# Chairy-neko/TinyRayTracing

Hardware: AMD Instinct MI355X
Metric: Mrays/s (higher is better)
Workload: dtype f32; 1 GPU; example-scenes-cg22 test/back Cornell-style box (26 triangles), 1920x1080, 256 spp; scene=back, width=1920, height=1080, spp=256, triangles=26, bvh_nodes=4, bvh_builder=auto, leaf_num=8, inner_node_bytes=64, overlap_passes=False, fixed_nee=False, tiling=single GPU

## Files before the change

tinyraytracing_amd/csrc/trt_api.hip:

```cpp
#include <hip/hip_runtime.h>

#include <dlfcn.h>

#include <algorithm>
#include <cstdio>
#include <cstdlib>
#include <atomic>
#include <limits>
#include <chrono>
#include <cstring>
#include <condition_variable>
#include <memory>
#include <mutex>
#include <string>
#include <thread>
#include <vector>

#include "trt.h"
#include "trt_kernels.h"
#include "trt_wide.h"
#include "trt_oct_build.h"

using namespace trtd;

// ... 14 lines not shown
            return fail(e_ == hipErrorOutOfMemory ? TRT_ENOMEM : TRT_EHIP, std::string(#expr) + ": " + hipGetErrorString(e_)); \
    } while (0)

constexpr uint32_t MAX_TRACE_BLOCKS = 8192;
constexpr uint32_t SPILL_STRIDE = MAX_TRACE_BLOCKS * TRT_TRACE_BLOCK;
constexpr uint32_t MAX_BOUNCES = TRT_MAX_PATH_DEPTH + 2;
constexpr uint32_t COUNT_STRIDE = (MAX_BOUNCES + 2 + 1023u) & ~1023u;
constexpr uint32_t COUNT_ROW_MIN = 16;
inline uint32_t countRows(uint32_t nl) { return std::max(COUNT_ROW_MIN, (nl + 3u + 15u) & ~15u); }
inline unsigned long long* pairCounter(uint32_t* d_counts, uint32_t rows, uint32_t b) { return reinterpret_cast<unsigned long long*>(d_counts + (size_t)(rows - 2u) * COUNT_STRIDE) + b; }
static_assert(TRT_MAX_SCENE_LIGHTS <= 65535u, "counter area");
constexpr uint32_t MAX_BVH_DEPTH = 256;
#ifndef TRT_DEFAULT_NODE_KIND
#define TRT_DEFAULT_NODE_KIND 1
#endif

struct DevBuf {
    void* p = nullptr;
    size_t bytes = 0;
    int ensure(size_t need)
    {
        if (need <= bytes) return TRT_OK;
        if (p) { (void)hipFree(p); p = nullptr; bytes = 0; }
        HIPC(hipMalloc(&p, need));
        bytes = need;
        return TRT_OK;
    }
    void release()
    {
        if (p) (void)hipFree(p);
        p = nullptr;
        bytes = 0;
    }
};

}

struct trt_handle {
    int device = 0;
    SceneDev sc{};
    std::vector<void*> scene_allocs;
    std::vector<uint32_t> light_mats;
    std::vector<LightBox> light_boxes;
    uint32_t depth = 0;
    uint32_t bvh2_depth = 0;
    uint32_t shade_tabs = 0;
    uint32_t shade_pad_lds = 0;
    const void* lds_image = nullptr;
    uint32_t lds_image_bytes = 0;
    uint32_t lds_tab[5] = {0, 0, 0, 0, 0};
    int trace_impl = 3;
    bool slim_walk = false;
    bool hit8 = false;
    int node_kind = 0;
    uint32_t oct_levels = 0;
    bool dbg = false;
    uint32_t rays_per_wave = 256, fill_blocks = 2048, max_blocks = 8192;
    uint32_t traceGrid(uint32_t n) const
    {
        uint32_t b = (n + TRT_TRACE_BLOCK - 1) / TRT_TRACE_BLOCK;
        if (rays_per_wave > 64) {
            const uint32_t want = (uint32_t)(((uint64_t)n + 4ull * rays_per_wave - 1) / (4ull * rays_per_wave));
            b = std::min(b, std::max(fill_blocks, want));
        }
        b = std::min(std::max(b, 8u), std::min(max_blocks, 8192u));
        return (b + 7u) & ~7u;
    }
    uint32_t tail_n = 131072;
    DevBuf arena, spill, small_buf, out_buf, io_buf;
    size_t spill_words_per_slot = 0;
    hipStream_t slot_streams[2] = {nullptr, nullptr};
    int n_slots = 2;
    uint32_t* pinned_counts = nullptr;
    uint32_t count_rows = COUNT_ROW_MIN;
    uint32_t slot_seq[2] = {0, 0};
    int fail_at_bounce = -1;
    std::vector<hipEvent_t> events;
    ~trt_handle()
    {
        for (void* p : scene_allocs) (void)hipFree(p);
        arena.release();
        spill.release();
        small_buf.release();
        out_buf.release();
        io_buf.release();
        for (hipEvent_t e : events) (void)hipEventDestroy(e);
        for (hipStream_t st : slot_streams) if (st) (void)hipStreamDestroy(st);
        if (pinned_counts) (void)hipHostFree(pinned_counts);
    }
};

namespace {

template <class T>
int upload(trt_handle* h, const T* src, size_t count, const T** dst)
{
    void* p = nullptr;
    const size_t bytes = (std::max<size_t>(count, 1) * sizeof(T) + 15) & ~(size_t)15;
    HIPC(hipMalloc(&p, bytes));
    h->scene_allocs.push_back(p);
    if (count) HIPC(hipMemcpy(p, src, count * sizeof(T), hipMemcpyHostToDevice));
    *dst = (const T*)p;
    return TRT_OK;
}

int validateBvh(const trt_scene* s, uint32_t* depth_out, unsigned threads = 1)
// ... 106 lines not shown

bool rowSelected(const trt_params* p, int y) { return p->row_mod <= 1 || ((y / p->row_block) % p->row_mod) == p->row_rem; }

uint32_t tailGrid(uint32_t n)
{
    uint32_t b = (n + TRT_TRACE_BLOCK - 1) / TRT_TRACE_BLOCK;
    b = std::min(std::max(b, 8u), MAX_TRACE_BLOCKS);
    return (b + 7u) & ~7u;
}
struct Timer {
    trt_handle* h;
    bool on;
    size_t used = 0;
    struct Span { int k; size_t e0, e1; };
    std::vector<Span> spans{};
    static constexpr size_t RESERVED = 3;
    hipEvent_t get(size_t i)
    {
        while (h->events.size() <= i) {
            hipEvent_t e;
            if (hipEventCreate(&e) != hipSuccess) return nullptr;
            h->events.push_back(e);
        }
        return h->events[i];
    }
    size_t mark(hipStream_t stream)
    {
        hipEvent_t e = get(RESERVED + used);
        if (e) (void)hipEventRecord(e, stream);
        return RESERVED + used++;
    }
    void begin(int k, hipStream_t stream) { if (on) spans.push_back({k, mark(stream), 0}); }
    void end(hipStream_t stream) { if (on) spans.back().e1 = mark(stream); }
    template <class F>
    void launch(int k, hipStream_t stream, trt_stats& st, F&& f)
    {
        begin(k, stream);
        f();
        end(stream);
        st.launches[k]++;
    }
};

using ClosestKernel = void (*)(SceneDev, RaySource, f4*, uint32_t, uint32_t*, uint32_t, DeviceStats*, RedoList);
using ShadowKernel = void (*)(SceneDev, ShadowQueue, uint32_t, uint32_t, f4*, uint32_t*, uint32_t, DeviceStats*, uint32_t, RedoList, LightBox);
using FixKernel = void (*)(SceneDev, RaySource, f4*, const f4*, uint32_t, f4*, uint32_t*, uint32_t, RedoList, uint32_t, DeviceStats*);
using ShadeKernel = void (*)(SceneDev, ShadeArgs);
using TailKernel = void (*)(SceneDev, TailArgs);

constexpr uint32_t OCT_LDS_LEVELS = 10;
int traversalOf(const trt_handle* h) { return h->trace_impl == 0 ? 0 : (h->node_kind == 1 ? 1 : (h->depth <= 16 ? 2 : 3)); }
ClosestKernel closestKernel(const trt_handle* h, bool count, int primary)
{
    if (h->trace_impl == 0 && h->hit8) {
        const ClosestKernel s[2][3] = {
            {k_trace_closest<false, 1, false, 0, 0, 0, true, true>, k_trace_closest<false, 1, false, 0, 1, 0, true, true>, k_trace_closest<false, 1, false, 0, PRIMARY_LIST, 0, true, true>},
            {k_trace_closest<true, 1, false, 0, 0, 0, true, true>, k_trace_closest<true, 1, false, 0, 1, 0, true, true>, k_trace_closest<true, 1, false, 0, PRIMARY_LIST, 0, true, true>}};
        return s[count][primary];
    }
    const ClosestKernel k[4][2][3] = {
        {{k_trace_closest<false, 1, false, 0, 0, 0>, k_trace_closest<false, 1, false, 0, 1, 0>, k_trace_closest<false, 1, false, 0, PRIMARY_LIST, 0>},
         {k_trace_closest<true, 1, false, 0, 0, 0>, k_trace_closest<true, 1, false, 0, 1, 0>, k_trace_closest<true, 1, false, 0, PRIMARY_LIST, 0>}},
        {{k_trace_closest<false, OCT_LDS_LEVELS, true, 3, 0, 1>, k_trace_closest<false, OCT_LDS_LEVELS, true, 3, 1, 1>, k_trace_closest<false, OCT_LDS_LEVELS, true, 3, PRIMARY_LIST, 1>},
         {k_trace_closest<true, OCT_LDS_LEVELS, true, 3, 0, 1>, k_trace_closest<true, OCT_LDS_LEVELS, true, 3, 1, 1>, k_trace_closest<true, OCT_LDS_LEVELS, true, 3, PRIMARY_LIST, 1>}},
        {{k_trace_closest<false, 16, false, 3, 0, 0>, k_trace_closest<false, 16, false, 3, 1, 0>, k_trace_closest<false, 16, false, 3, PRIMARY_LIST, 0>},
         {k_trace_closest<true, 16, false, 3, 0, 0>, k_trace_closest<true, 16, false, 3, 1, 0>, k_trace_closest<true, 16, false, 3, PRIMARY_LIST, 0>}},
        {{k_trace_closest<false, TRT_LDS_STACK_MAX, true, 3, 0, 0>, k_trace_closest<false, TRT_LDS_STACK_MAX, true, 3, 1, 0>, k_trace_closest<false, TRT_LDS_STACK_MAX, true, 3, PRIMARY_LIST, 0>},
         {k_trace_closest<true, TRT_LDS_STACK_MAX, true, 3, 0, 0>, k_trace_closest<true, TRT_LDS_STACK_MAX, true, 3, 1, 0>, k_trace_closest<true, TRT_LDS_STACK_MAX, true, 3, PRIMARY_LIST, 0>}}};
    return k[traversalOf(h)][count][primary];
}
ShadowKernel shadowKernel(const trt_handle* h, bool count)
{
    if (h->trace_impl == 0 && h->slim_walk) return count ? k_trace_shadow<true, 1, false, 0, 0, true> : k_trace_shadow<false, 1, false, 0, 0, true>;
    const ShadowKernel k[4][2] = {{k_trace_shadow<false, 1, false, 0, 0>, k_trace_shadow<true, 1, false, 0, 0>},
                                  {k_trace_shadow<false, OCT_LDS_LEVELS, true, 3, 1>, k_trace_shadow<true, OCT_LDS_LEVELS, true, 3, 1>},
                                  {k_trace_shadow<false, 16, false, 3, 0>, k_trace_shadow<true, 16, false, 3, 0>},
                                  {k_trace_shadow<false, TRT_LDS_STACK_MAX, true, 3, 0>, k_trace_shadow<true, TRT_LDS_STACK_MAX, true, 3, 0>}};
    return k[traversalOf(h)][count];
}
FixKernel fixKernel(const trt_handle* h, bool shadow, int primary)
{
    const FixKernel k[4] = {k_trace_fix<false, 0, 0>, k_trace_fix<false, 1, 0>, k_trace_fix<false, PRIMARY_LIST, 0>, k_trace_fix<true, false, 0>};
    return h->trace_impl == 0 ? nullptr : k[shadow ? 3 : primary];
}
ClosestKernel queryKernel(const trt_handle* h, int query)
{
    const bool occ = query == QUERY_OCCLUDED;
    if (h->trace_impl == 0 && h->hit8 && !occ) return k_trace_query<QUERY_CLOSEST, true, 1, false, 0, 0, true, true>;
    if (h->trace_impl == 0 && h->slim_walk && occ) return k_trace_query<QUERY_OCCLUDED, true, 1, false, 0, 0, false, true>;
    const ClosestKernel k[4][2] = {{k_trace_query<QUERY_CLOSEST, true, 1, false, 0, 0>, k_trace_query<QUERY_OCCLUDED, true, 1, false, 0, 0>},
                                   {k_trace_query<QUERY_CLOSEST, true, OCT_LDS_LEVELS, true, 3, 1>, k_trace_query<QUERY_OCCLUDED, true, OCT_LDS_LEVELS, true, 3, 1>},
                                   {k_trace_query<QUERY_CLOSEST, true, 16, false, 3, 0>, k_trace_query<QUERY_OCCLUDED, true, 16, false, 3, 0>},
                                   {k_trace_query<QUERY_CLOSEST, true, TRT_LDS_STACK_MAX, true, 3, 0>, k_trace_query<QUERY_OCCLUDED, true, TRT_LDS_STACK_MAX, true, 3, 0>}};
    return k[traversalOf(h)][occ];
}
FixKernel queryFixKernel(const trt_handle* h, int query)
{
    if (h->trace_impl == 0) return nullptr;
    return query == QUERY_OCCLUDED ? k_trace_fix<true, 0, 0, QUERY_OCCLUDED> : k_trace_fix<false, 0, 0, QUERY_CLOSEST>;
}
ShadeKernel shadeKernel(uint32_t tabs, int lights, bool list, bool hit8)
{
    if (hit8) {
        const ShadeKernel s[2][3] = {
            {k_shade<31u, SHADE_ONE, false, TRT_SHADE1_BLOCK, TRT_SHADE1_WAVES, true>, k_shade<31u, SHADE_FEW, false, TRT_SHADEN_BLOCK, TRT_SHADEN_WAVES, true>,
             k_shade<31u, SHADE_MANY, false, TRT_SHADEN_BLOCK, TRT_SHADEN_WAVES, true>},
// ... 233 lines not shown
        if (int e = upload(h.get(), im.cum.data(), im.cum.size(), &h->sc.light_cum)) return e;
    if (int e = upload(h.get(), im.tex.data(), im.tex.size(), &h->sc.textures)) return e;
    if (int e = upload(h.get(), im.tex_bytes.data(), im.tex_bytes.size(), &h->sc.tex_bytes)) return e;
    lap("uploads");
    h->sc.n_tris = s->n_tris;
    h->sc.n_nodes = s->n_nodes;
    h->sc.n_lights = s->n_lights;
    h->sc.light0_area = s->n_lights ? s->lights[0].area : 0.0f;
    h->sc.leaf_alpha = im.leaf_alpha;
    h->sc.cull_alpha = im.cull_alpha;
    h->sc.cam = s->camera;
    for (uint32_t i = 0; i < s->n_lights; ++i) h->light_mats.push_back((uint32_t)s->lights[i].mat);
    {
        const uint32_t want[5] = {(uint32_t)(s->n_materials * sizeof(MaterialDev)), (uint32_t)(s->n_lights * sizeof(LightDev)),
                                  h->sc.light_cum ? (uint32_t)(s->n_light_tris * sizeof(float)) : 0u, (uint32_t)(s->n_light_tris * sizeof(LightTriDev)),
                                  s->n_tris <= 64 ? (uint32_t)(s->n_tris * sizeof(TriShade)) : 0u};
        uint32_t used = 0;
        for (int k = 0; k < 5; ++k) {
            const uint32_t padded = (want[k] + 15u) & ~15u;
            if (want[k] && used + padded <= TRT_SHADE_LDS_TABLE_BYTES) { h->lds_tab[k] = want[k]; used += padded; }
        }
        if (std::getenv("TRT_SHADE_NO_LDS")) h->lds_tab[0] = h->lds_tab[1] = h->lds_tab[2] = h->lds_tab[3] = h->lds_tab[4] = 0;
        if (std::getenv("TRT_SHADE_NO_LDS_TRIS")) h->lds_tab[4] = 0;
        uint32_t have = 0;
        for (int k = 0; k < 5; ++k) have |= h->lds_tab[k] ? (1u << k) : 0u;
        h->shade_tabs = 0;
        for (uint32_t m : {31u, 15u, 7u, 3u})
            if ((have & m) == m) { h->shade_tabs = m; break; }
        if (im.dbg)
            std::fprintf(stderr, "trt_create: k_shade tables %u (lds bytes: materials %u, lights %u, cdf %u, light tris %u, shading tris %u)\n", h->shade_tabs,
                         h->lds_tab[0], h->lds_tab[1], h->lds_tab[2], h->lds_tab[3], h->lds_tab[4]);
        const void* src[5] = {h->sc.materials, h->sc.lights, h->sc.light_cum, h->sc.light_tris, h->sc.tri_shade};
        size_t total = 0;
        for (int k = 0; k < 5; ++k)
            if (h->shade_tabs >> k & 1u) total += (h->lds_tab[k] + 15u) & ~15u;
        if (total) {
            void* img = nullptr;
            HIPC(hipMalloc(&img, total));
            h->scene_allocs.push_back(img);
            size_t off = 0;
            for (int k = 0; k < 5; ++k)
                if (h->shade_tabs >> k & 1u) {
                    const size_t padded = (h->lds_tab[k] + 15u) & ~15u;
                    HIPC(hipMemcpy((char*)img + off, src[k], padded, hipMemcpyDeviceToDevice));
                    off += padded;
                }
            h->lds_image = img;
            h->lds_image_bytes = (uint32_t)total;
        }
    }
    h->slim_walk = h->trace_impl == 0 && s->n_tris <= 64;
    if (const char* e = std::getenv("TRT_SLIM_WALK")) h->slim_walk = h->slim_walk && std::atoi(e) != 0;
    h->hit8 = h->slim_walk && h->shade_tabs == 31u;
    if (im.dbg) std::fprintf(stderr, "trt_create: slim walk %d, 8-byte hit records %d\n", (int)h->slim_walk, (int)h->hit8);

    const uint32_t stack_levels = std::max(h->depth, h->bvh2_depth + 2u);
    uint32_t spill_levels = stack_levels > (uint32_t)TRT_LDS_STACK_MAX ? stack_levels - TRT_LDS_STACK_MAX + 1 : 1;
    if (h->node_kind == 1 && h->oct_levels > OCT_LDS_LEVELS) spill_levels = std::max(spill_levels, 2u * (h->oct_levels - OCT_LDS_LEVELS + 1));
    h->spill_words_per_slot = (size_t)spill_levels * SPILL_STRIDE;
    if (int e = h->spill.ensure(h->spill_words_per_slot * 2 * sizeof(uint32_t))) return e;
    for (hipStream_t& st : h->slot_streams) HIPC(hipStreamCreateWithFlags(&st, hipStreamNonBlocking));
    h->count_rows = countRows(h->sc.n_lights);
    const size_t pinned_words = 2 * (2 * (size_t)h->count_rows + 16);
    HIPC(hipHostMalloc((void**)&h->pinned_counts, pinned_words * sizeof(uint32_t), hipHostMallocDefault));
    std::memset(h->pinned_counts, 0, pinned_words * sizeof(uint32_t));
    if (const char* e = std::getenv("TRT_SLOTS")) h->n_slots = std::atoi(e) >= 2 ? 2 : 1;
    if (const char* e = std::getenv("TRT_TEST_FAIL_AT_BOUNCE")) h->fail_at_bounce = std::atoi(e);
    if (const char* e = std::getenv("TRT_SHADE_PAD_LDS")) {
        h->shade_pad_lds = std::min(100000u, (uint32_t)std::strtoul(e, nullptr, 10));
        for (uint32_t tabs : {31u, 15u, 7u, 3u, 0u})
            for (bool list : {false, true})
                for (int lights : {SHADE_ONE, SHADE_FEW, SHADE_MANY})
                    for (bool hit8 : {false, true})
                        if (!hit8 || tabs == 31u)
                            (void)hipFuncSetAttribute(reinterpret_cast<const void*>(shadeKernel(tabs, lights, list, hit8)), hipFuncAttributeMaxDynamicSharedMemorySize, (int)h->shade_pad_lds);
    }

    *out = h.release();
    return TRT_OK;
}
}

extern "C" {

const char* trt_last_error(void) { return g_err.c_str(); }
int trt_abi_version(void) { return TRT_ABI_VERSION; }

int trt_rows_selected(const trt_params* p)
{
    if (!p) return -1;
    int n = 0;
    for (int y = p->y0; y < p->y1; ++y) n += rowSelected(p, y) ? 1 : 0;
    return n;
}

int trt_create(const trt_scene* s, int device, trt_handle** out)
{
    if (!s || !out) return fail(TRT_EINVAL, "trt_create: null argument");
    *out = nullptr;
    SceneImage im;
    if (int e = buildSceneImage(s, im)) return e;
    return createOnDevice(im, device, out);
}

void trt_destroy(trt_handle* h)
{
    if (!h) return;
// ... 1019 lines not shown
```

tinyraytracing_amd/csrc/trt_kernels.h:

```cpp
#pragma once
#include <hip/hip_runtime.h>
#include <type_traits>

#include "trt_path.h"
#include "trt_oct.h"

namespace trtd {

#ifndef TRT_TRACE_MINWAVES
#define TRT_TRACE_MINWAVES 0
#endif
#if TRT_TRACE_MINWAVES > 0
#define TRT_TRACE_BOUNDS __launch_bounds__(256, TRT_TRACE_MINWAVES)
#else
#define TRT_TRACE_BOUNDS __launch_bounds__(256)
#endif
constexpr int TRT_TRACE_BLOCK = 256;
#ifndef TRT_LDS_STACK_MAX_LEVELS
#define TRT_LDS_STACK_MAX_LEVELS 16
#endif
constexpr int TRT_LDS_STACK_MAX = TRT_LDS_STACK_MAX_LEVELS;
#ifndef TRT_SHADE1_BLOCK
#define TRT_SHADE1_BLOCK 512
#endif
// ... 172 lines not shown
        float u = 0.f, v = 0.f;
        if (best_tri >= 0) {
            float t, un, vn, det;
            if (triTest(sc.tri_isect[best_tri], o, d, t, un, vn, det)) { u = un / det; v = vn / det; }
        }
        TRT_STQ(8, hit + idx, mk4(best_t, u2f((uint32_t)best_tri), u, v));
    } else if (any ? best_tri < 0 : (best_tri >= 0 && (best_flags >> 8) == light_mat)) {
        const f4 w = TRT_LDQ(16, sw + idx);
        f4 L = TRT_LDQ(32, Lacc + pid);
        L.x = L.x + w.x; L.y = L.y + w.y; L.z = L.z + w.z;
        TRT_STQ(32, Lacc + pid, L);
    }
}

template <bool SHADOW, bool OCT = false, int QUERY = QUERY_NONE>
__device__ __forceinline__ bool checkedStore(const SceneDev& sc, f3 o, f3 d, f3 inv, float best_t, int32_t best_tri, uint32_t best_flags, uint32_t idx, uint32_t pid,
                                             f4* __restrict__ hit, const f4* __restrict__ sw, uint32_t light_mat, f4* __restrict__ Lacc, bool any)
{
    const bool special = raySpecial(inv);
    const uint32_t tri = best_tri >= 0 ? (uint32_t)best_tri : 0u;
    const f4 ba = sc.leaf_box[2 * (size_t)tri], bb = sc.leaf_box[2 * (size_t)tri + 1];
    if (!SHADOW) {
        const TriIsect T = sc.tri_isect[tri];
        float e;
        const bool pass = boxTest(ba.x, ba.y, ba.z, ba.w, bb.x, bb.y, o, inv, e);
        if (special || (best_tri >= 0 && ((OCT && !pass) || best_t < trt_leaf_floor(e, sc.leaf_alpha)))) return true;
        float u = 0.f, v = 0.f;
        if (best_tri >= 0) {
            float t, un, vn, det;
            if (triTest(T, o, d, t, un, vn, det)) { u = un / det; v = vn / det; }
        }
        TRT_STQ(8, hit + idx, mk4(QUERY == QUERY_CLOSEST && best_tri < 0 ? TRT_INF : best_t, u2f((uint32_t)best_tri), u, v));
    } else if constexpr (QUERY == QUERY_OCCLUDED) {
        float e;
        const bool pass = boxTest(ba.x, ba.y, ba.z, ba.w, bb.x, bb.y, o, inv, e);
        if (special || (best_tri >= 0 && ((OCT && !pass) || best_t < trt_leaf_floor(e, sc.leaf_alpha)))) return true;
        reinterpret_cast<uint8_t*>(hit)[idx] = best_tri >= 0 ? 1u : 0u;
    } else {
        const bool vis = any ? best_tri < 0 : (best_tri >= 0 && (best_flags >> 8) == light_mat);
        f4 w = mk4(0, 0, 0, 0), L = w;
        if (vis) { w = TRT_LDQ(16, sw + idx); L = TRT_LDQ(32, Lacc + pid); }
        float e;
        const bool pass = boxTest(ba.x, ba.y, ba.z, ba.w, bb.x, bb.y, o, inv, e);
        if (special || (best_tri >= 0 && ((OCT && !pass) || best_t < trt_leaf_floor(e, sc.leaf_alpha)))) return true;
        if (vis) {
            L.x = L.x + w.x; L.y = L.y + w.y; L.z = L.z + w.z;
            TRT_STQ(32, Lacc + pid, L);
        }
    }
    return false;
}

constexpr int TRT_PEND_SLOTS = 4;
template <bool COUNT, int STRIDE, bool GLM, bool FLAGS_LDS = false>
__device__ __forceinline__ void uniformWalkImpl(const SceneDev& sc, f3 o, f3 d, f3 inv, bool valid, bool special, f4* __restrict__ my_pend, float& best_t, int32_t& best_tri,
                                                uint32_t& best_flags, uint32_t& n_inner, uint32_t& n_tri, const uint32_t* tri_flags = nullptr)
{
    const uint32_t n_nodes = sc.n_nodes;
    uint32_t reach = valid ? 1u : 0u;
    uint32_t n_pend = 0;
    auto flush = [&]() {
        for (uint32_t s = 0; ballotb(s < n_pend) != 0ull; ++s) {
            if (s < n_pend) {
                const f4 e = my_pend[s * STRIDE];
                const float t = e.x / e.y;
                if (!(t < TRT_T_MIN) && !(t < e.w)) {
                    const uint32_t pk = f2u(e.z);
                    const int32_t j = (int32_t)(pk & 0xFFu);
                    const uint32_t fl = FLAGS_LDS ? tri_flags[j] : f2u(sc.tri_isect[j].c.z);
                    bool take = t < best_t;
                    if (t == best_t && best_tri >= 0) {
                        const bool em = (fl & 1u) != 0, bem = (best_flags & 1u) != 0;
                        const uint32_t first = (pk >> 8) & 0xFFu, cnt = pk >> 16;
                        const bool same_leaf = (uint32_t)best_tri >= first && (uint32_t)best_tri < first + cnt;
                        take = same_leaf ? em : (em ? (!bem || j < best_tri) : (!bem && j > best_tri));
                    }
                    if (take) { best_t = t; best_tri = j; best_flags = fl; }
                }
            }
        }
        n_pend = 0;
    };
    for (uint32_t ni = 0; ni < n_nodes; ++ni) {
        const bool at = (reach >> ni) & 1u;
        if (ballotb(at) == 0ull) continue;
        const f4* np4 = reinterpret_cast<const f4*>(sc.nodes + ni);
        const f4 q0 = np4[0], q1 = np4[1], q2 = np4[2], q3 = np4[3];
        if (COUNT && at) n_inner++;
        float e0 = 0.0f, e1 = 0.0f;
        bool h0 = at && boxTest(q0.x, q0.y, q0.z, q0.w, q1.x, q1.y, o, inv, e0);
        bool h1 = at && boxTest(q1.z, q1.w, q2.x, q2.y, q2.z, q2.w, o, inv, e1);
        if (GLM) {
            float g0, g1;
            const bool s0 = boxTestGlm(q0.x, q0.y, q0.z, q0.w, q1.x, q1.y, o, inv, g0), s1 = boxTestGlm(q1.z, q1.w, q2.x, q2.y, q2.z, q2.w, o, inv, g1);
            if (special) { h0 = at && s0; h1 = at && s1; e0 = g0; e1 = g1; }
        }
        const float f0 = trt_leaf_floor(e0, sc.leaf_alpha), f1 = trt_leaf_floor(e1, sc.leaf_alpha);
        const uint32_t child[2] = {f2u(q3.x), f2u(q3.y)};
        const bool hc[2] = {h0, h1};
#pragma unroll
        for (int c = 0; c < 2; ++c) {
            const uint32_t ref = child[c];
            if (!(ref & TRT_LEAF_BIT)) {
                reach |= hc[c] ? (1u << ref) : 0u;
                continue;
            }
            const unsigned long long m_hc = ballotb(hc[c]);
            if (m_hc == 0ull) continue;
            const uint32_t first = TRT_LEAF_FIRST(ref), count = TRT_LEAF_COUNT(ref);
            for (uint32_t k = 0; k < count; ++k) {
                const TriIsect T = sc.tri_isect[first + k];
                if (COUNT && hc[c]) n_tri++;
                float tn, un, vn, det;
                bool ok_det, ok_in;
                triCandidateParts(T, o, d, tn, un, vn, det, ok_det, ok_in);
                const bool cand = ok_det && ok_in && hc[c];
                if ((ballotb(ok_det) & ballotb(ok_in) & m_hc & ballotb(n_pend == (uint32_t)TRT_PEND_SLOTS)) != 0ull) flush();
                if (cand) {
                    my_pend[n_pend * STRIDE] = mk4(tn, det, u2f((first + k) | (first << 8) | (count << 16)), c == 0 ? f0 : f1);
                    n_pend++;
                }
            }
        }
    }
    flush();
}
template <bool COUNT, int STRIDE = TRT_TRACE_BLOCK>
__device__ __forceinline__ void uniformWalk(const SceneDev& sc, f3 o, f3 d, bool valid, f4* __restrict__ my_pend, float& best_t, int32_t& best_tri,
                                            uint32_t& best_flags, uint32_t& n_inner, uint32_t& n_tri)
{
    const f3 inv = mk3(1.0f / d.x, 1.0f / d.y, 1.0f / d.z);
    const bool special = valid && raySpecial(inv);
    if (ballotb(special) != 0ull) uniformWalkImpl<COUNT, STRIDE, true>(sc, o, d, inv, valid, special, my_pend, best_t, best_tri, best_flags, n_inner, n_tri);
    else uniformWalkImpl<COUNT, STRIDE, false>(sc, o, d, inv, valid, false, my_pend, best_t, best_tri, best_flags, n_inner, n_tri);
}
// ... 35 lines not shown
        if (lane == 0 && n_parked) atomicAdd(&stats->redo_rays, n_parked);
        n_parked = 0;
    };
    for (uint32_t base = lb * TRT_TRACE_BLOCK; base < n; base += stride) {
        const uint32_t i = base + threadIdx.x;
        const bool valid = i < n;
        const uint32_t ii = valid ? i : n - 1;
        f4 a, b;
        fetchRay<PRIMARY>(sc, src, ii, a, b);
        const f3 o = mk3(a.x, a.y, a.z), d = mk3(a.w, b.x, b.y);
        const f3 inv = mk3(1.0f / d.x, 1.0f / d.y, 1.0f / d.z);
        float best_t = bounded ? b.w : TRT_INF;
        int32_t best_tri = -1;
        uint32_t best_flags = 0u;
        uniformWalkImpl<COUNT, TRT_TRACE_BLOCK, false, PIPE>(sc, o, d, inv, valid, false, my_pend, best_t, best_tri, best_flags, n_inner, n_tri, s_flags);
        const bool special = valid && raySpecial(inv);
        if (valid && !special) storeResult<SHADOW, HIT8, QUERY>(sc, o, d, best_t, best_tri, best_flags, i, SHADOW ? f2u(b.z) : 0u, hit, sw, light_mat, Lacc, any);
        const unsigned long long m_sp = ballotb(special);
        if (m_sp != 0ull) {
            const uint32_t at = n_parked + (uint32_t)__popcll(m_sp & ((1ull << lane) - 1ull));
            if (special && at < 128u) my_parked[at] = i;
            n_parked += (uint32_t)__popcll(m_sp);
        }
    }
    if (n_parked != 0u && n_parked <= 128u) rewalk();
    else if (n_parked > 128u) {
        for (uint32_t base = lb * TRT_TRACE_BLOCK; base < n; base += stride) {
            const uint32_t i = base + threadIdx.x;
            const bool valid = i < n;
            f4 a, b;
            fetchRay<PRIMARY>(sc, src, valid ? i : n - 1, a, b);
            const f3 o = mk3(a.x, a.y, a.z), d = mk3(a.w, b.x, b.y);
            const f3 inv = mk3(1.0f / d.x, 1.0f / d.y, 1.0f / d.z);
            const bool special = valid && raySpecial(inv);
            if (ballotb(special) == 0ull) continue;
            float best_t = bounded ? b.w : TRT_INF;
            int32_t best_tri = -1;
            uint32_t best_flags = 0u;
            uint32_t ni = 0, nt = 0;
            uniformWalkImpl<false, TRT_TRACE_BLOCK, true, PIPE>(sc, o, d, inv, special, special, my_pend, best_t, best_tri, best_flags, ni, nt, s_flags);
            if (special) storeResult<SHADOW, HIT8, QUERY>(sc, o, d, best_t, best_tri, best_flags, i, SHADOW ? f2u(b.z) : 0u, hit, sw, light_mat, Lacc, any);
        }
        if (lane == 0) atomicAdd(&stats->redo_rays, n_parked);
    }
    if (COUNT) {
        const unsigned long long si = waveSum(n_inner), st = waveSum(n_tri);
        if ((threadIdx.x & 63) == 0) {
            atomicAdd(&stats->inner_visits[SHADOW ? 1 : 0], si);
            atomicAdd(&stats->tri_tests[SHADOW ? 1 : 0], st);
        }
    }
}


template <bool SHADOW, bool COUNT, int DEPTH, bool SPILL, int IMPL, int PRIMARY, int NK, int QUERY = QUERY_NONE>
__device__ __forceinline__ void traceQueuePersistent(const SceneDev& sc, const RaySource& src, uint32_t n, f4* __restrict__ hit,
                                           const f4* __restrict__ sw, uint32_t light_mat, f4* __restrict__ Lacc, uint32_t* __restrict__ spill,
                                           uint32_t spill_stride, DeviceStats* stats, uint32_t* smem, bool any_flag, RedoList redo)
{
    LdsStack<DEPTH, SPILL> stk;
    stk.lds = smem + threadIdx.x;
    stk.spill = spill + (size_t)blockIdx.x * TRT_TRACE_BLOCK + threadIdx.x;
    stk.spill_stride = spill_stride;
    const bool any = SHADOW && (QUERY == QUERY_OCCLUDED || any_flag);
    const uint32_t lane = threadIdx.x & 63u;
    const unsigned long long lower = (1ull << lane) - 1ull;
    const uint32_t n_waves = gridDim.x * (TRT_TRACE_BLOCK / 64);
    const uint32_t wave = xcdSwizzle(blockIdx.x, gridDim.x) * (TRT_TRACE_BLOCK / 64) + (threadIdx.x >> 6);
    const uint32_t per = (n + n_waves - 1) / n_waves;
    const unsigned long long w0 = (unsigned long long)wave * per;
    uint32_t next = (uint32_t)__builtin_amdgcn_readfirstlane((int)(w0 < n ? w0 : n));
    const uint32_t end = (uint32_t)__builtin_amdgcn_readfirstlane((int)((w0 + per) < n ? (w0 + per) : n));

    uint32_t cur = TRT_REF_IDLE, idx = 0, pid = 0;
    int sp = 0;
    f3 o = mk3(0, 0, 0), d = mk3(0, 0, 0), inv = mk3(0, 0, 0);
    float best_t = TRT_INF;
    int32_t best_tri = -1;
    uint32_t best_flags = 0;
    uint32_t lk = 0;
    float lt = TRT_INF;
    int32_t li = -1;
    uint32_t lflags = 0;
    TraceProbe pr;

    for (;;) {
        const bool working = cur < TRT_REF_DONE;
        const unsigned long long m_work = ballotb(working);
        const unsigned long long m_done = ballotb(cur == TRT_REF_DONE);
        const unsigned long long m_free = ~m_work;
        const bool can_fill = next < end;
        if (m_work == 0ull || (m_done != 0ull && (uint32_t)__popcll(can_fill ? m_free : m_done) >= sc.refill_min)) {
            if (cur == TRT_REF_DONE) {
                if (checkedStore<SHADOW, false, QUERY>(sc, o, d, inv, best_t, best_tri, best_flags, idx, pid, hit, sw, light_mat, Lacc, any)) redo.idx[atomicAdd(redo.count, 1u)] = idx;
                cur = TRT_REF_IDLE;
            }
            if (can_fill) {
                const uint32_t rank = (uint32_t)__popcll(m_free & lower);
                if (!working && next + rank < end) {
                    idx = next + rank;
                    f4 a, b;
                    fetchRay<PRIMARY>(sc, src, idx, a, b);
                    o = mk3(a.x, a.y, a.z);
                    d = mk3(a.w, b.x, b.y);
                    if (SHADOW) pid = f2u(b.z);
                    inv = mk3(1.0f / d.x, 1.0f / d.y, 1.0f / d.z);
// ... 174 lines not shown
            }
        }
        if (adv) {
            if (sp != 0 && !(any && best_tri >= 0)) ng = stk.pop(--sp);
            else if (SHADOW && !any && best_tri < 0 && best_t < TRT_INF) { best_t = TRT_INF; ng.x = 0u; ng.y = 0x80000000u; }
            else ng.y = 0u;
        }
    }
    if (COUNT) {
        const unsigned long long si = waveSum(pr.n_inner), st = waveSum(pr.n_tri), wi = waveSum(pr.wave_inner), wt = waveSum(pr.wave_tri);
        if (lane == 0) {
            atomicAdd(&stats->inner_visits[SHADOW ? 1 : 0], si);
            atomicAdd(&stats->tri_tests[SHADOW ? 1 : 0], st);
            atomicAdd(&stats->wave_inner_steps, wi);
            atomicAdd(&stats->wave_leaf_steps, wt);
            atomicAdd(&stats->census_inner, (unsigned long long)pr.c_in);
            atomicAdd(&stats->census_leaf, (unsigned long long)pr.c_lf);
            atomicAdd(&stats->census_done, (unsigned long long)pr.c_done);
            atomicAdd(&stats->census_iters, (unsigned long long)pr.c_it);
        }
    }
}

template <bool SHADOW, bool COUNT, int DEPTH, bool SPILL, int IMPL, int PRIMARY, int NK, bool HIT8 = false, bool PIPE = false, int QUERY = QUERY_NONE>
__device__ __forceinline__ void traceQueue(const SceneDev& sc, const RaySource& src, uint32_t n, f4* __restrict__ hit,
                                           const f4* __restrict__ sw, uint32_t light_mat, f4* __restrict__ Lacc, uint32_t* __restrict__ spill,
                                           uint32_t spill_stride, DeviceStats* stats, uint32_t* smem, bool any_flag, RedoList redo, const LightBox& lbox)
{
    static_assert(IMPL == 0 || !(HIT8 || PIPE), "8-byte hit records and the flags in LDS belong to the wave-uniform walk");
    if constexpr (IMPL == 0) traceQueueUniform<SHADOW, COUNT, PRIMARY, HIT8, PIPE, QUERY>(sc, src, n, hit, sw, light_mat, Lacc, stats, any_flag, reinterpret_cast<f4*>(smem));
    else if constexpr (NK == 1) traceQueuePersistentOct<SHADOW, COUNT, DEPTH, SPILL, PRIMARY, QUERY>(sc, src, n, hit, sw, light_mat, Lacc, spill, spill_stride, stats, smem, any_flag, redo, lbox);
    else traceQueuePersistent<SHADOW, COUNT, DEPTH, SPILL, IMPL, PRIMARY, NK, QUERY>(sc, src, n, hit, sw, light_mat, Lacc, spill, spill_stride, stats, smem, any_flag, redo);
}

template <bool COUNT, int DEPTH, bool SPILL, int IMPL, int PRIMARY, int NK, bool HIT8 = false, bool PIPE = false>
__global__ TRT_TRACE_BOUNDS void k_trace_closest(SceneDev sc, RaySource src, f4* __restrict__ hit, uint32_t n,
                                                 uint32_t* __restrict__ spill, uint32_t spill_stride, DeviceStats* stats, RedoList redo)
{
    __shared__ __attribute__((aligned(16))) uint32_t smem[IMPL == 0 ? TRT_PEND_SLOTS * 4 * TRT_TRACE_BLOCK : (NK == 1 ? 2 : 1) * DEPTH * TRT_TRACE_BLOCK];
    const LightBox nobox = {{0.f, 0.f, 0.f}, {0.f, 0.f, 0.f}};
    traceQueue<false, COUNT, DEPTH, SPILL, IMPL, PRIMARY, NK, HIT8, PIPE>(sc, src, n, hit, nullptr, 0u, nullptr, spill, spill_stride, stats, smem, false, redo, nobox);
}

template <bool COUNT, int DEPTH, bool SPILL, int IMPL, int NK, bool PIPE = false>
__global__ TRT_TRACE_BOUNDS void k_trace_shadow(SceneDev sc, ShadowQueue sq, uint32_t n, uint32_t light_mat, f4* __restrict__ Lacc,
                                                uint32_t* __restrict__ spill, uint32_t spill_stride, DeviceStats* stats, uint32_t any, RedoList redo, LightBox lbox)
{
    __shared__ __attribute__((aligned(16))) uint32_t smem[IMPL == 0 ? TRT_PEND_SLOTS * 4 * TRT_TRACE_BLOCK : (NK == 1 ? 2 : 1) * DEPTH * TRT_TRACE_BLOCK];
    RaySource src;
    src.ra = sq.sa;
    src.rb = sq.sb;
    src.s0 = 0;
    traceQueue<true, COUNT, DEPTH, SPILL, IMPL, false, NK, false, PIPE>(sc, src, n, nullptr, sq.sw, light_mat, Lacc, spill, spill_stride, stats, smem, any != 0u, redo, lbox);
}

template <int QUERY, bool COUNT, int DEPTH, bool SPILL, int IMPL, int NK, bool HIT8 = false, bool PIPE = false>
__global__ TRT_TRACE_BOUNDS void k_trace_query(SceneDev sc, RaySource src, f4* __restrict__ hit, uint32_t n,
                                               uint32_t* __restrict__ spill, uint32_t spill_stride, DeviceStats* stats, RedoList redo)
{
    static_assert(QUERY == QUERY_CLOSEST || QUERY == QUERY_OCCLUDED, "k_trace_closest serves the unbounded closest hit");
    __shared__ __attribute__((aligned(16))) uint32_t smem[IMPL == 0 ? TRT_PEND_SLOTS * 4 * TRT_TRACE_BLOCK : (NK == 1 ? 2 : 1) * DEPTH * TRT_TRACE_BLOCK];
    const LightBox nobox = {{0.f, 0.f, 0.f}, {0.f, 0.f, 0.f}};
    constexpr bool OCC = QUERY == QUERY_OCCLUDED;
    traceQueue<OCC, COUNT, DEPTH, SPILL, IMPL, 0, NK, HIT8, PIPE, QUERY>(sc, src, n, hit, nullptr, 0u, nullptr, spill, spill_stride, stats, smem, OCC, redo, nobox);
}

constexpr uint32_t TRT_FIX_BLOCKS = 32;
template <bool SHADOW, int PRIMARY, int NK, int QUERY = QUERY_NONE>
__global__ __launch_bounds__(TRT_TRACE_BLOCK) void k_trace_fix(SceneDev sc, RaySource src, f4* __restrict__ hit, const f4* __restrict__ sw, uint32_t light_mat,
                                                               f4* __restrict__ Lacc, uint32_t* __restrict__ spill, uint32_t spill_stride, RedoList redo, uint32_t any_flag,
                                                               DeviceStats* stats)
{
    __shared__ __attribute__((aligned(16))) uint32_t smem[TRT_LDS_STACK_MAX * TRT_TRACE_BLOCK];
    const uint32_t n = *redo.count;
    if (n == 0u) return;
    {
        LdsStack<TRT_LDS_STACK_MAX, true> stk;
        stk.lds = smem + threadIdx.x;
        stk.spill = spill + (size_t)blockIdx.x * TRT_TRACE_BLOCK + threadIdx.x;
        stk.spill_stride = spill_stride;
        const bool any = SHADOW && (QUERY == QUERY_OCCLUDED || any_flag != 0u);
        for (uint32_t k = blockIdx.x * TRT_TRACE_BLOCK + threadIdx.x; k < n; k += gridDim.x * TRT_TRACE_BLOCK) {
            const uint32_t i = redo.idx[k];
            f4 a, b;
            fetchRay<PRIMARY>(sc, src, i, a, b);
            const f3 o = mk3(a.x, a.y, a.z), d = mk3(a.w, b.x, b.y);
            uint32_t ni = 0, nt = 0;
            const f3 inv = mk3(1.0f / d.x, 1.0f / d.y, 1.0f / d.z);
            const float t_init = (SHADOW || QUERY != QUERY_NONE) ? b.w : TRT_INF;
            Hit h = (raySpecial(inv) && rayOnABoxPlane(sc, o, inv))
                        ? traceClosestBvh2Glm<LdsStack<TRT_LDS_STACK_MAX, true>, false>(sc, o, d, stk, ni, nt, t_init, any)
                        : traceClosestPass<LdsStack<TRT_LDS_STACK_MAX, true>, false, NK, true>(sc, o, d, stk, ni, nt, t_init, any, SHADOW && !any);
            if (QUERY == QUERY_CLOSEST && !(h.t < b.w)) h.tri = -1;
            storeResult<SHADOW, false, QUERY>(sc, o, d, h.t, h.tri, h.flags, i, SHADOW ? f2u(b.z) : 0u, hit, sw, light_mat, Lacc, any);
        }
    }
    __syncthreads();
    if (threadIdx.x == 0) {
        __threadfence();
        if (atomicAdd(redo.count + 1, 1u) + 1u == gridDim.x) {
            atomicAdd(&stats->redo_rays, n);
            redo.count[1] = 0u;
            redo.count[0] = 0u;
        }
    }
}
// ... 548 lines not shown
```

Before: 23120 Mrays/s.

## Add binned closest-hit walk that sorts rays by leaf-hit mask before triangle tests

Adds a new closest-hit kernel for tiny scenes. A first pass over the box tree records which leaves each ray reaches. Each wave then counting-sorts 256 rays by that leaf-mask key in LDS and runs the triangle tests on the sorted order, so lanes in a wave visit the same leaves and branch less. Rays with special directions are parked and retraced afterwards with the existing uniform walk. It is on by default for non-primary bounces when 8-byte hit records are active, at the cost of walking the box tree twice, extra LDS traffic and a waves-per-EU hint.

```diff
diff --git a/tinyraytracing_amd/csrc/trt_api.hip b/tinyraytracing_amd/csrc/trt_api.hip
--- a/tinyraytracing_amd/csrc/trt_api.hip
+++ b/tinyraytracing_amd/csrc/trt_api.hip
@@ -90,6 +90,7 @@
     int trace_impl = 3;
     bool slim_walk = false;
     bool hit8 = false;
+    bool bin_walk = false;
     int node_kind = 0;
     uint32_t oct_levels = 0;
     bool dbg = false;
@@ -302,6 +303,7 @@
 int traversalOf(const trt_handle* h) { return h->trace_impl == 0 ? 0 : (h->node_kind == 1 ? 1 : (h->depth <= 16 ? 2 : 3)); }
 ClosestKernel closestKernel(const trt_handle* h, bool count, int primary)
 {
+    if (h->bin_walk && primary == 0) return count ? k_trace_closest_binned<true> : k_trace_closest_binned<false>;
     if (h->trace_impl == 0 && h->hit8) {
         const ClosestKernel s[2][3] = {
             {k_trace_closest<false, 1, false, 0, 0, 0, true, true>, k_trace_closest<false, 1, false, 0, 1, 0, true, true>, k_trace_closest<false, 1, false, 0, PRIMARY_LIST, 0, true, true>},
@@ -641,7 +643,9 @@
     h->slim_walk = h->trace_impl == 0 && s->n_tris <= 64;
     if (const char* e = std::getenv("TRT_SLIM_WALK")) h->slim_walk = h->slim_walk && std::atoi(e) != 0;
     h->hit8 = h->slim_walk && h->shade_tabs == 31u;
-    if (im.dbg) std::fprintf(stderr, "trt_create: slim walk %d, 8-byte hit records %d\n", (int)h->slim_walk, (int)h->hit8);
+    h->bin_walk = h->hit8;
+    if (const char* e = std::getenv("TRT_BIN_WALK")) h->bin_walk = h->bin_walk && std::atoi(e) != 0;
+    if (im.dbg) std::fprintf(stderr, "trt_create: slim walk %d, 8-byte hit records %d, binned walk %d\n", (int)h->slim_walk, (int)h->hit8, (int)h->bin_walk);
 
     const uint32_t stack_levels = std::max(h->depth, h->bvh2_depth + 2u);
     uint32_t spill_levels = stack_levels > (uint32_t)TRT_LDS_STACK_MAX ? stack_levels - TRT_LDS_STACK_MAX + 1 : 1;
diff --git a/tinyraytracing_amd/csrc/trt_kernels.h b/tinyraytracing_amd/csrc/trt_kernels.h
--- a/tinyraytracing_amd/csrc/trt_kernels.h
+++ b/tinyraytracing_amd/csrc/trt_kernels.h
@@ -248,6 +248,51 @@
 }
 
 constexpr int TRT_PEND_SLOTS = 4;
+template <int STRIDE, bool FLAGS_LDS>
+__device__ __forceinline__ void flushPending(const SceneDev& sc, const f4* __restrict__ my_pend, uint32_t& n_pend, float& best_t, int32_t& best_tri,
+                                             uint32_t& best_flags, const uint32_t* tri_flags)
+{
+    for (uint32_t s = 0; ballotb(s < n_pend) != 0ull; ++s) {
+        if (s < n_pend) {
+            const f4 e = my_pend[s * STRIDE];
+            const float t = e.x / e.y;
+            if (!(t < TRT_T_MIN) && !(t < e.w)) {
+                const uint32_t pk = f2u(e.z);
+                const int32_t j = (int32_t)(pk & 0xFFu);
+                const uint32_t fl = FLAGS_LDS ? tri_flags[j] : f2u(sc.tri_isect[j].c.z);
+                bool take = t < best_t;
+                if (t == best_t && best_tri >= 0) {
+                    const bool em = (fl & 1u) != 0, bem = (best_flags & 1u) != 0;
+                    const uint32_t first = (pk >> 8) & 0xFFu, cnt = pk >> 16;
+                    const bool same_leaf = (uint32_t)best_tri >= first && (uint32_t)best_tri < first + cnt;
+                    take = same_leaf ? em : (em ? (!bem || j < best_tri) : (!bem && j > best_tri));
+                }
+                if (take) { best_t = t; best_tri = j; best_flags = fl; }
+            }
+        }
+    }
+    n_pend = 0;
+}
+template <bool COUNT, int STRIDE, bool FLAGS_LDS>
+__device__ __forceinline__ void walkLeaf(const SceneDev& sc, f3 o, f3 d, bool hc, unsigned long long m_hc, uint32_t ref, float floor, f4* __restrict__ my_pend,
+                                         uint32_t& n_pend, float& best_t, int32_t& best_tri, uint32_t& best_flags, uint32_t& n_tri, const uint32_t* tri_flags)
+{
+    const uint32_t first = TRT_LEAF_FIRST(ref), count = TRT_LEAF_COUNT(ref);
+    for (uint32_t k = 0; k < count; ++k) {
+        const TriIsect T = sc.tri_isect[first + k];
+        if (COUNT && hc) n_tri++;
+        float tn, un, vn, det;
+        bool ok_det, ok_in;
+        triCandidateParts(T, o, d, tn, un, vn, det, ok_det, ok_in);
+        const bool cand = ok_det && ok_in && hc;
+        if ((ballotb(ok_det) & ballotb(ok_in) & m_hc & ballotb(n_pend == (uint32_t)TRT_PEND_SLOTS)) != 0ull)
+            flushPending<STRIDE, FLAGS_LDS>(sc, my_pend, n_pend, best_t, best_tri, best_flags, tri_flags);
+        if (cand) {
+            my_pend[n_pend * STRIDE] = mk4(tn, det, u2f((first + k) | (first << 8) | (count << 16)), floor);
+            n_pend++;
+        }
+    }
+}
 template <bool COUNT, int STRIDE, bool GLM, bool FLAGS_LDS = false>
 __device__ __forceinline__ void uniformWalkImpl(const SceneDev& sc, f3 o, f3 d, f3 inv, bool valid, bool special, f4* __restrict__ my_pend, float& best_t, int32_t& best_tri,
                                                 uint32_t& best_flags, uint32_t& n_inner, uint32_t& n_tri, const uint32_t* tri_flags = nullptr)
@@ -255,28 +300,7 @@
     const uint32_t n_nodes = sc.n_nodes;
     uint32_t reach = valid ? 1u : 0u;
     uint32_t n_pend = 0;
-    auto flush = [&]() {
-        for (uint32_t s = 0; ballotb(s < n_pend) != 0ull; ++s) {
-            if (s < n_pend) {
-                const f4 e = my_pend[s * STRIDE];
-                const float t = e.x / e.y;
-                if (!(t < TRT_T_MIN) && !(t < e.w)) {
-                    const uint32_t pk = f2u(e.z);
-                    const int32_t j = (int32_t)(pk & 0xFFu);
-                    const uint32_t fl = FLAGS_LDS ? tri_flags[j] : f2u(sc.tri_isect[j].c.z);
-                    bool take = t < best_t;
-                    if (t == best_t && best_tri >= 0) {
-                        const bool em = (fl & 1u) != 0, bem = (best_flags & 1u) != 0;
-                        const uint32_t first = (pk >> 8) & 0xFFu, cnt = pk >> 16;
-                        const bool same_leaf = (uint32_t)best_tri >= first && (uint32_t)best_tri < first + cnt;
-                        take = same_leaf ? em : (em ? (!bem || j < best_tri) : (!bem && j > best_tri));
-                    }
-                    if (take) { best_t = t; best_tri = j; best_flags = fl; }
-                }
-            }
-        }
-        n_pend = 0;
-    };
+    auto flush = [&]() { flushPending<STRIDE, FLAGS_LDS>(sc, my_pend, n_pend, best_t, best_tri, best_flags, tri_flags); };
     for (uint32_t ni = 0; ni < n_nodes; ++ni) {
         const bool at = (reach >> ni) & 1u;
         if (ballotb(at) == 0ull) continue;
@@ -418,6 +442,211 @@
     }
 }
 
+#define TRT_BIN_WAVES __attribute__((amdgpu_waves_per_eu(8)))
+#ifndef TRT_BIN_GROUP
+#define TRT_BIN_GROUP 4
+#endif
+constexpr uint32_t TRT_BIN_KEYS = 256;
+__device__ __forceinline__ void waveSync()
+{
+    __builtin_amdgcn_fence(__ATOMIC_RELEASE, "wavefront");
+    __builtin_amdgcn_wave_barrier();
+    __builtin_amdgcn_fence(__ATOMIC_ACQUIRE, "wavefront");
+}
+template <bool COUNT>
+__device__ __forceinline__ void traceQueueBinned(const SceneDev& sc, const RaySource& src, uint32_t n, f4* __restrict__ hit, DeviceStats* stats, f4* __restrict__ pend)
+{
+    constexpr uint32_t B = TRT_TRACE_BLOCK, G = TRT_BIN_GROUP;
+    static_assert(G * 64u == TRT_BIN_KEYS && TRT_PEND_SLOTS == 4, "one wave sorts 256 rays; its four 256-word pieces of the candidate queue hold the sort");
+    uint32_t n_inner = 0, n_tri = 0;
+    const uint32_t lb = xcdSwizzle(blockIdx.x, gridDim.x);
+    const uint32_t stride = gridDim.x * B;
+    f4* my_pend = pend + threadIdx.x;
+    const uint32_t lane = threadIdx.x & 63u;
+    uint32_t* piece = reinterpret_cast<uint32_t*>(pend) + 4u * 64u * (threadIdx.x >> 6);
+    uint32_t* s_hist = piece;
+    uint32_t* x_idx = piece + 4u * B;
+    uint32_t* x_lo = piece + 8u * B;
+    uint32_t* x_hi = piece + 12u * B;
+    __shared__ uint32_t s_flags[64];
+    __shared__ uint32_t s_parked[2 * B];
+    uint32_t* my_parked = s_parked + (threadIdx.x >> 6) * 128u;
+    const uint32_t n_nodes = sc.n_nodes;
+    bool l0 = false, l1 = false;
+    if (lane < n_nodes) {
+        const f4 q3 = reinterpret_cast<const f4*>(sc.nodes + lane)[3];
+        l0 = (f2u(q3.x) & TRT_LEAF_BIT) != 0u;
+        l1 = (f2u(q3.y) & TRT_LEAF_BIT) != 0u;
+    }
+    const unsigned long long lf0 = ballotb(l0), lf1 = ballotb(l1);
+    const uint32_t run = ((uint32_t)(__popcll(lf0) + __popcll(lf1)) + 7u) >> 3;
+    if (threadIdx.x < (sc.n_tris < 64u ? sc.n_tris : 64u)) s_flags[threadIdx.x] = f2u(sc.tri_isect[threadIdx.x].c.z);
+    __syncthreads();
+    uint32_t n_parked = 0;
+    for (uint32_t base0 = lb * B; base0 < n; base0 += G * stride) {
+        reinterpret_cast<uint4*>(s_hist)[lane] = make_uint4(0u, 0u, 0u, 0u);
+        waveSync();
+#pragma unroll 1
+        for (uint32_t j = 0; j < G; ++j) {
+            const uint32_t i = base0 + j * stride + threadIdx.x;
+            const bool valid = i < n;
+            f4 a, b;
+            fetchRay<0>(sc, src, valid ? i : n - 1, a, b);
+            const f3 o = mk3(a.x, a.y, a.z), d = mk3(a.w, b.x, b.y);
+            const f3 inv = mk3(1.0f / d.x, 1.0f / d.y, 1.0f / d.z);
+            uint32_t reach = valid ? 1u : 0u;
+            unsigned long long mask = 0ull;
+            for (uint32_t ni = 0; ni < n_nodes; ++ni) {
+                const bool at = (reach >> ni) & 1u;
+                if (ballotb(at) == 0ull) continue;
+                const f4* np4 = reinterpret_cast<const f4*>(sc.nodes + ni);
+                const f4 q0 = np4[0], q1 = np4[1], q2 = np4[2], q3 = np4[3];
+                if (COUNT && at) n_inner++;
+                float e0, e1;
+                const bool h0 = at && boxTest(q0.x, q0.y, q0.z, q0.w, q1.x, q1.y, o, inv, e0);
+                const bool h1 = at && boxTest(q1.z, q1.w, q2.x, q2.y, q2.z, q2.w, o, inv, e1);
+                const unsigned long long below = (1ull << ni) - 1ull;
+                const uint32_t leaf0 = (uint32_t)(__popcll(lf0 & below) + __popcll(lf1 & below));
+                const uint32_t ref0 = f2u(q3.x), ref1 = f2u(q3.y);
+                if (ref0 & TRT_LEAF_BIT) mask |= h0 ? (1ull << leaf0) : 0ull;
+                else reach |= h0 ? (1u << ref0) : 0u;
+                if (ref1 & TRT_LEAF_BIT) mask |= h1 ? (1ull << (leaf0 + ((ref0 & TRT_LEAF_BIT) ? 1u : 0u))) : 0ull;
+                else reach |= h1 ? (1u << ref1) : 0u;
+            }
+            uint32_t key = (uint32_t)mask & (TRT_BIN_KEYS - 1u);
+            if (run > 1u) {
+                key = 0u;
+                for (uint32_t k = 0; k < 8u; ++k) key |= ((mask >> (k * run)) & ((1ull << run) - 1ull)) != 0ull ? (1u << k) : 0u;
+            }
+            x_idx[j * 64u + lane] = key | (atomicAdd(&s_hist[key], 1u) << 8);
+            x_lo[j * 64u + lane] = (uint32_t)mask;
+            x_hi[j * 64u + lane] = (uint32_t)(mask >> 32);
+        }
+        waveSync();
+        const uint4 h = reinterpret_cast<const uint4*>(s_hist)[lane];
+        const uint32_t own = h.x + h.y + h.z + h.w;
+        uint32_t incl = own;
+        for (int off = 1; off < 64; off <<= 1) {
+            const uint32_t up = __shfl_up(incl, off);
+            if ((int)lane >= off) incl += up;
+        }
+        const uint32_t ex = incl - own;
+        reinterpret_cast<uint4*>(s_hist)[lane] = make_uint4(ex, ex + h.x, ex + h.x + h.y, ex + h.x + h.y + h.z);
+        uint32_t rk[G];
+        unsigned long long msk[G];
+#pragma unroll
+        for (uint32_t j = 0; j < G; ++j) {
+            rk[j] = x_idx[j * 64u + lane];
+            msk[j] = (unsigned long long)x_lo[j * 64u + lane] | ((unsigned long long)x_hi[j * 64u + lane] << 32);
+        }
+        waveSync();
+#pragma unroll
+        for (uint32_t j = 0; j < G; ++j) {
+            const uint32_t r = s_hist[rk[j] & 0xFFu] + (rk[j] >> 8);
+            x_idx[r] = base0 + j * stride + threadIdx.x;
+            x_lo[r] = (uint32_t)msk[j];
+            x_hi[r] = (uint32_t)(msk[j] >> 32);
+        }
+        waveSync();
+        uint32_t sidx[G];
+        unsigned long long smask[G];
+#pragma unroll
+        for (uint32_t j = 0; j < G; ++j) {
+            sidx[j] = x_idx[j * 64u + lane];
+            smask[j] = (unsigned long long)x_lo[j * 64u + lane] | ((unsigned long long)x_hi[j * 64u + lane] << 32);
+        }
+        waveSync();
+#pragma unroll 1
+        for (uint32_t j = 0; j < G; ++j) {
+            const uint32_t i = sidx[0];
+            const unsigned long long mask = smask[0];
+#pragma unroll
+            for (uint32_t k = 0; k + 1 < G; ++k) { sidx[k] = sidx[k + 1]; smask[k] = smask[k + 1]; }
+            const bool valid = i < n;
+            f4 a, b;
+            fetchRay<0>(sc, src, valid ? i : n - 1, a, b);
+            const f3 o = mk3(a.x, a.y, a.z), d = mk3(a.w, b.x, b.y);
+            const f3 inv = mk3(1.0f / d.x, 1.0f / d.y, 1.0f / d.z);
+            float best_t = TRT_INF;
+            int32_t best_tri = -1;
+            uint32_t best_flags = 0u;
+            uint32_t n_pend = 0;
+            for (uint32_t ni = 0; ni < n_nodes; ++ni) {
+                const bool c0 = (lf0 >> ni) & 1ull, c1 = (lf1 >> ni) & 1ull;
+                if (!c0 && !c1) continue;
+                const unsigned long long below = (1ull << ni) - 1ull;
+                const uint32_t leaf0 = (uint32_t)(__popcll(lf0 & below) + __popcll(lf1 & below));
+                const bool hc0 = c0 && ((mask >> leaf0) & 1ull);
+                const bool hc1 = c1 && ((mask >> (leaf0 + (c0 ? 1u : 0u))) & 1ull);
+                const unsigned long long m0 = ballotb(hc0), m1 = ballotb(hc1);
+                if ((m0 | m1) == 0ull) continue;
+                const f4* np4 = reinterpret_cast<const f4*>(sc.nodes + ni);
+                const f4 q0 = np4[0], q1 = np4[1], q2 = np4[2], q3 = np4[3];
+                if (m0 != 0ull) {
+                    float e = 0.0f;
+                    if (hc0) boxTest(q0.x, q0.y, q0.z, q0.w, q1.x, q1.y, o, inv, e);
+                    walkLeaf<COUNT, B, true>(sc, o, d, hc0, m0, f2u(q3.x), trt_leaf_floor(e, sc.leaf_alpha), my_pend, n_pend, best_t, best_tri, best_flags, n_tri, s_flags);
+                }
+                if (m1 != 0ull) {
+                    float e = 0.0f;
+                    if (hc1) boxTest(q1.z, q1.w, q2.x, q2.y, q2.z, q2.w, o, inv, e);
+                    walkLeaf<COUNT, B, true>(sc, o, d, hc1, m1, f2u(q3.y), trt_leaf_floor(e, sc.leaf_alpha), my_pend, n_pend, best_t, best_tri, best_flags, n_tri, s_flags);
+                }
+            }
+            flushPending<B, true>(sc, my_pend, n_pend, best_t, best_tri, best_flags, s_flags);
+            const bool special = valid && raySpecial(inv);
+            if (valid && !special) storeResult<false, true>(sc, o, d, best_t, best_tri, best_flags, i, 0u, hit, nullptr, 0u, nullptr, false);
+            const unsigned long long m_sp = ballotb(special);
+            if (m_sp != 0ull) {
+                const uint32_t at = n_parked + (uint32_t)__popcll(m_sp & ((1ull << lane) - 1ull));
+                if (special && at < 128u) my_parked[at] = i;
+                n_parked += (uint32_t)__popcll(m_sp);
+            }
+        }
+        waveSync();
+    }
+    if (n_parked != 0u && n_parked <= 128u) {
+        for (uint32_t pb = 0; pb < n_parked; pb += 64u) {
+            const bool valid = pb + lane < n_parked;
+            const uint32_t i = my_parked[valid ? pb + lane : 0u];
+            f4 a, b;
+            fetchRay<0>(sc, src, i, a, b);
+            const f3 o = mk3(a.x, a.y, a.z), d = mk3(a.w, b.x, b.y);
+            float best_t = TRT_INF;
+            int32_t best_tri = -1;
+            uint32_t best_flags = 0u;
+            uint32_t ni = 0, nt = 0;
+            uniformWalkImpl<false, B, true, true>(sc, o, d, mk3(1.0f / d.x, 1.0f / d.y, 1.0f / d.z), valid, valid, my_pend, best_t, best_tri, best_flags, ni, nt, s_flags);
+            if (valid) storeResult<false, true>(sc, o, d, best_t, best_tri, best_flags, i, 0u, hit, nullptr, 0u, nullptr, false);
+        }
+        if (lane == 0) atomicAdd(&stats->redo_rays, n_parked);
+    } else if (n_parked > 128u) {
+        for (uint32_t base = lb * B; base < n; base += stride) {
+            const uint32_t i = base + threadIdx.x;
+            const bool valid = i < n;
+            f4 a, b;
+            fetchRay<0>(sc, src, valid ? i : n - 1, a, b);
+            const f3 o = mk3(a.x, a.y, a.z), d = mk3(a.w, b.x, b.y);
+            const f3 inv = mk3(1.0f / d.x, 1.0f / d.y, 1.0f / d.z);
+            const bool special = valid && raySpecial(inv);
+            if (ballotb(special) == 0ull) continue;
+            float best_t = TRT_INF;
+            int32_t best_tri = -1;
+            uint32_t best_flags = 0u;
+            uint32_t ni = 0, nt = 0;
+            uniformWalkImpl<false, B, true, true>(sc, o, d, inv, special, special, my_pend, best_t, best_tri, best_flags, ni, nt, s_flags);
+            if (special) storeResult<false, true>(sc, o, d, best_t, best_tri, best_flags, i, 0u, hit, nullptr, 0u, nullptr, false);
+        }
+        if (lane == 0) atomicAdd(&stats->redo_rays, n_parked);
+    }
+    if (COUNT) {
+        const unsigned long long si = waveSum(n_inner), st = waveSum(n_tri);
+        if (lane == 0) {
+            atomicAdd(&stats->inner_visits[0], si);
+            atomicAdd(&stats->tri_tests[0], st);
+        }
+    }
+}
 
 template <bool SHADOW, bool COUNT, int DEPTH, bool SPILL, int IMPL, int PRIMARY, int NK, int QUERY = QUERY_NONE>
 __device__ __forceinline__ void traceQueuePersistent(const SceneDev& sc, const RaySource& src, uint32_t n, f4* __restrict__ hit,
@@ -698,6 +927,14 @@
     src.rb = sq.sb;
     src.s0 = 0;
     traceQueue<true, COUNT, DEPTH, SPILL, IMPL, false, NK, false, PIPE>(sc, src, n, nullptr, sq.sw, light_mat, Lacc, spill, spill_stride, stats, smem, any != 0u, redo, lbox);
+}
+
+template <bool COUNT>
+__global__ TRT_TRACE_BOUNDS TRT_BIN_WAVES void k_trace_closest_binned(SceneDev sc, RaySource src, f4* __restrict__ hit, uint32_t n,
+                                                                      uint32_t* __restrict__ spill, uint32_t spill_stride, DeviceStats* stats, RedoList redo)
+{
+    __shared__ __attribute__((aligned(16))) uint32_t smem[TRT_PEND_SLOTS * 4 * TRT_TRACE_BLOCK];
+    traceQueueBinned<COUNT>(sc, src, n, hit, stats, reinterpret_cast<f4*>(smem));
 }
 
 template <int QUERY, bool COUNT, int DEPTH, bool SPILL, int IMPL, int NK, bool HIT8 = false, bool PIPE = false>
```

New measurement: 23800 Mrays/s, median of 6. +2.9%, better.
